# OSOceanAcoustics/echopype

Hardware: AMD Instinct MI355X
Metric: range-samples/sec through compute_Sv->compute_MVBS (higher is better)
Workload: dtype f64; 1 GPU; cfg5: EK60 CW 4x2000000x4096 in ping_time tiles, compute_Sv -> compute_MVBS(20s x 1m), Sv+MVBS out; tiles=8 x 250000 pings over 1 rank(s), route=compute_Sv -> compute_MVBS('1m','20s') per tile, collective=none at 1 rank, tile_streams=2

## Files before the change

### echopype_amd/csrc/epa_internal.h

```cpp
#pragma once
#include <cstdlib>
#include <hip/hip_runtime.h>

#include <atomic>

#include <cmath>
#include <cstdarg>
#include <cstdint>
#include <cstdio>

#include "echopype_amd.h"

namespace epa {

void set_error(const char* fmt, ...);

#define EPA_CHECK_ARG(cond, ...)       \
  do {                                 \
    if (!(cond)) {                     \
      ::epa::set_error(__VA_ARGS__);   \
      return EPA_EINVAL;               \
    }                                  \
  } while (0)

#define EPA_CHECK_HIP(expr)                                                              \
  do {                                                                                   \
    hipError_t _e = (expr);                                                              \
    if (_e != hipSuccess) {                                                              \
      ::epa::set_error("%s failed: %s (%s:%d)", #expr, hipGetErrorString(_e), __FILE__,  \
                       __LINE__);                                                        \
      return EPA_EHIP;                                                                   \
    }                                                                                    \
  } while (0)

template <typename T>
struct type_tag {
  using type = T;
};

template <typename T>
constexpr int dtype_of = sizeof(T) == 8 ? EPA_F64 : EPA_F32;

inline bool is_real(int dtype) { return dtype == EPA_F32 || dtype == EPA_F64; }

#define EPA_CHECK_REAL(who, dtype) EPA_CHECK_ARG(::epa::is_real(dtype), "%s: bad dtype %d", who, dtype)
#define EPA_CHECK_REAL_OUT(who, dtype) EPA_CHECK_ARG(::epa::is_real(dtype), "%s: bad output dtype %d", who, dtype)

template <typename F>
int dispatch_real(const char* who, int dtype, F&& f) {
  if (dtype == EPA_F64) return f(type_tag<double>{});
  if (dtype == EPA_F32) return f(type_tag<float>{});
  set_error("%s: bad dtype %d", who, dtype);
  return EPA_EINVAL;
}

extern std::atomic<bool> g_trace_on;
void note_launch(const char* what);
void note_range_stats_filled(int filled);

void note_seen(const char* what);

inline int check_launch(const char* what) {
  if (g_trace_on.load(std::memory_order_relaxed)) note_launch(what);
  note_seen(what);
  hipError_t e = hipGetLastError();
  if (e != hipSuccess) {
    set_error("launch of %s failed: %s", what, hipGetErrorString(e));
    return EPA_EHIP;
  }
  return EPA_OK;
}

constexpr int kBlock = 256;
constexpr int kMinmaxMaxGrid = 1024;

inline bool al16(const void* p) { return p == nullptr || (reinterpret_cast<uintptr_t>(p) & 15u) == 0; }

template <typename T>
struct M;
template <>
struct M<double> {
  static __device__ __forceinline__ double log10(double x) { return ::log10(x); }
  static __device__ __forceinline__ double exp10(double x) { return ::exp10(x); }
  static __device__ __forceinline__ double nan() { return __builtin_nan(""); }
};
template <>
struct M<float> {
  static __device__ __forceinline__ float log10(float x) { return ::log10f(x); }
  static __device__ __forceinline__ float exp10(float x) { return ::exp10f(x); }
  static __device__ __forceinline__ float nan() { return __builtin_nanf(""); }
};

struct CoefRow {
  double ra, rb, r0, shift, alpha2, A0, g, d;
};
static_assert(sizeof(CoefRow) == EPA_NCOEF * sizeof(double), "coef row layout");

__device__ __forceinline__ int xcd_contiguous(int x, int n) {
  const int per = n >> 3;
  return x < per * 8 ? (x & 7) * per + (x >> 3) : x;
}
inline bool xcd_map_enabled() {
  static const bool on = [] {
    const char* e = getenv("EPA_XCD_MAP");
    return !(e && e[0] == '0');
  }();
  return on;
}

__device__ __forceinline__ int range_bin_index(double x, double bin, double inv_bin, int nbins,
                                               bool closed_right) {
  if (!(x == x)) return -1;
  double t = x * inv_bin;
  if (!(t > -2.0)) return -1;
  if (t > (double)nbins + 2.0) return -1;
  int i;
  if (!closed_right) {
    i = (int)floor(t);
    if (x < (double)i * bin) --i;
    else if (x >= (double)(i + 1) * bin) ++i;
  } else {
    i = (int)ceil(t) - 1;
    if (x <= (double)i * bin) --i;
    else if (x > (double)(i + 1) * bin) ++i;
  }
  return (i >= 0 && i < nbins) ? i : -1;
}

__device__ __forceinline__ double row_range(const CoefRow& r, int s) {
  return ((double)s * r.ra) * r.rb + r.r0;
}

__device__ __forceinline__ double depth_of(double scale, double offset, double range) {
#pragma clang fp contract(off)
  const double prod = scale * range;
  return offset + prod;
}
__device__ __forceinline__ float depth_of(float scale, float offset, float range) {
#pragma clang fp contract(off)
  const float prod = scale * range;
  return offset + prod;
}

namespace scratch {
size_t sv_power_stats_workspace(long long S, long long, long long);
size_t depth_rows_workspace(long long, long long, long long);
size_t nanminmax_workspace(long long, long long, long long);
size_t range_step_mean_workspace(long long C, long long P, long long);
size_t sv_complex_cw_stats_workspace(long long, long long, long long);
size_t sv_complex_fft_workspace(long long W, long long P, long long S);
size_t splitbeam_complex_fft_workspace(long long n, long long, long long);
size_t sv_mvbs_fused_depth_stats(long long, long long, long long);
size_t apply_masks_workspace(long long, long long, long long);
size_t pool_sv_sum_ws(long long C, long long P, long long S);
size_t pool_sv_cnt_ws(long long C, long long P, long long S);
size_t pool_sv_value_ws_mean(long long C, long long P, long long S);
size_t pool_sv_value_ws_median(long long C, long long S, long long);
size_t nasc_workspace(long long C, long long n_dbins, long long n_rbins);
size_t seafloor_state(long long, long long, long long);
size_t seafloor_angle_mask_work(long long P, long long R, long long);
size_t seafloor_median_hist(long long, long long, long long);
size_t shoal_state(long long, long long, long long);
size_t shoal_echoview_link_queue(long long, long long, long long);
size_t transient_fielding_todo(long long C, long long P, long long);
size_t transient_fielding_count(long long, long long, long long);
size_t transient_matecho_s_hi(long long C, long long P, long long);
size_t transient_matecho_flag(long long C, long long P, long long);
size_t time_rebuild_tile_workspace(long long N, long long, long long);
size_t regrid_mask_out(long long G, long long n_tbins, long long n_rbins);
}

#define EPA_CHECK_SCRATCH(who, what, used, have)                                                              \
  EPA_CHECK_ARG((size_t)(used) <= (size_t)(have), "%s: internal error: the launch plan writes %zu bytes of %s, sized %zu", \
                who, (size_t)(used), what, (size_t)(have))

}

int epa_rows_piece_launch(const float* mask_raw, const void* x, const double* coef, const double* scale,
                          const double* offset, long long rows, int S, void* out, int dtype, double* workspace,
                          double* stats_out, hipStream_t st);
int epa_minmax_final(const double* part, int nparts, double* out, hipStream_t st);
int epa_minmax_keys_init(unsigned long long* keys, hipStream_t st);
int epa_minmax_keys_decode(double* keys, hipStream_t st);

int epa_fused_fast_path(const void* raw, int raw_is_i16, const int32_t* n_valid, const double* coef,
                        int C, int P, int S, double nspread,
                        unsigned cal_flags, const int32_t* bin_start, int n_tbins, double range_bin,
                        int n_rbins, unsigned bin_flags, double fill_value, void* sv_out,
                        void* mvbs_out, void* sum_out, uint32_t* cnt_out, int dtype,
                        size_t lds_bytes, unsigned cnt_off, unsigned long long* rmax_key,
                        unsigned long long* rstat, const double* dscale, const double* doffset, void* depth_out,
                        hipStream_t st);
int epa_mvbs_rows_fast_path(const void* sv, const double* coef, int C, int P, int S, const int32_t* bin_start,
                            int n_tbins, double range_bin, int n_rbins, int as_stored, double fill_value,
                            void* mvbs_out, void* sum_out, uint32_t* cnt_out, int dtype, size_t lds_bytes,
                            unsigned cnt_off, hipStream_t st);
int epa_chain_fast_pass1(const float* raw, const double* coef, const double* alpha2, int C, int P, int S,
                         double nspread, int ping_num, int rsn, int ping_phase, double noise_max, void* sv_out,
                         double* noise_out, double* edge_sum_out, uint32_t* edge_cnt_out,
                         unsigned long long* rmax_key, unsigned long long* rstat, int dtype, hipStream_t st);
int epa_chain_fast_pass2(const float* raw, const double* coef, const double* alpha2, const double* noise, int C,
                         int P, int S, double nspread, int ping_num, int ping_phase, double snr,
                         const int32_t* bin_start, int n_tbins, double range_bin, int n_rbins, double fill_value,
                         void* noise_out, void* corr_out, void* mvbs_out, void* sum_out, uint32_t* cnt_out, int dtype,
                         size_t lds_acc_bytes, unsigned cnt_off, unsigned long long* mm_keys, hipStream_t st);
```

### echopype_amd/csrc/fused_sv_mvbs.hip

```cpp
#include <hip/amd_detail/amd_hip_unsafe_atomics.h>

#include <cstdlib>
#include <type_traits>

#include "fast_math.h"
#include "ordered_key.h"
#include "sample_math.h"

namespace epa_fused {

constexpr int VEC = 4;
constexpr int kChunk = epa::kBlock * VEC;

struct Args {
  int P, S, n_tbins, n_rbins;
  double range_bin, inv_range_bin;
  double nspread, fill_value;
  unsigned guard, mask_range, skipna, closed_right;
  unsigned cnt_off, tab_off;
  unsigned long long* rmax_key;
  unsigned long long* rstat;
  int xcd_map;
  int flagged_only;
  const double* dscale;
  const double* doffset;
  void* depth_out;
};

using epa::kKeyNoMax;
using epa::kKeyNoMin;
using epa::key_value;
using epa::lds_add;
using epa::ordered_key;
using epa::vmax_num;
using epa::vmin_num;

template <typename T>
__device__ __noinline__ T log10_slow(T x) {
  return epa::M<T>::log10(x);
}

template <typename T>
struct Column {
  double sra;
  double blo, bhi;
  T nL;
  T acc_sum;
  int acc_rb;
  uint32_t acc_cnt;
  __device__ __forceinline__ void init() {
    sra = 0.0; blo = 1.0; bhi = 0.0; nL = epa::M<T>::nan(); acc_sum = (T)0; acc_rb = -1; acc_cnt = 0u;
  }
  __device__ __forceinline__ void flush(T* lsum, uint32_t* lcnt, uint32_t n_clean) {
    const uint32_t n = acc_cnt + n_clean;
    if (acc_rb >= 0 && n > 0u) {
      lds_add(lsum + acc_rb, acc_sum);
      atomicAdd(lcnt + acc_rb, n);
    }
  }
  __device__ __forceinline__ void rebin(double x, bool valid, double bin, double inv_bin, int n_rbins, T* lsum,
                                        uint32_t* lcnt, uint32_t n_clean) {
    const int rb = valid ? epa::range_bin_index(x, bin, inv_bin, n_rbins, false) : -1;
    if (rb != acc_rb) {
      flush(lsum, lcnt, n_clean);
      acc_rb = rb;
      acc_sum = (T)0;
      acc_cnt = 0u - n_clean;
    }
    blo = rb >= 0 ? (double)rb * bin : 1.0;
    bhi = rb >= 0 ? (double)(rb + 1) * bin : 0.0;
  }
};

__device__ __forceinline__ double lin_bins(double u, const double* __restrict__ tab) {
  constexpr double K256 = 85.04135922911648, Z = 0.0027076061740622863;
  constexpr double C1 = Z, C2 = Z * Z / 2.0, C3 = Z * Z * Z / 6.0;
  const double t = u * K256;
  const double m = __builtin_rint(t);
  const double r = fma(u, K256, -m);
  double p = fma(r, C3, C2);
  p = fma(p, r, C1);
  p = fma(p, r, 1.0);
  const int mi = __double2int_rz(m);
  return ldexp(p * tab[mi & 255], mi >> 8);
}
__device__ __forceinline__ float lin_bins(float u, const double*) { return ::exp10f(u * 0.1f); }

template <typename T, bool STATS>
__device__ __forceinline__ T process_sample(Column<T>& c, float raw, const epa::CoefRow& r, double r0v, T g, T a2,
                                            T A0v, T nL, T nspread, double bin, double inv_bin, int n_rbins,
                                            const double* tab, T* lsum, uint32_t* lcnt, double& xmax, double& xmin,
                                            unsigned& nnan, uint32_t n_clean) {
  const T NaN = epa::M<T>::nan();
  const double x = fma(c.sra, r.rb, r0v);
  if (STATS) {
    if (raw == raw) {
      xmax = vmax_num(xmax, x);
      xmin = vmin_num(xmin, x);
    }
    nnan += (unsigned)__builtin_popcountll(__ballot(raw != raw));
  }
  const double rtd = x - r.shift;
  const T rt = (T)rtd;
  const bool pos = rtd > 0.0;
  T s1 = fma(g, (T)raw, nL);
  if (pos & !(nL > -(T)__builtin_inf()))
    s1 = fma(g, (T)raw, nspread * (log10_slow<T>(rt) - log10_slow<T>((T)(r.ra * r.rb))));
  s1 = pos ? s1 : NaN;
  const T sv = s1 + fma(a2, rt, A0v);
  const T v = epa::lin_from_db_lean(sv, tab);
  const bool same = (x >= c.blo) & (x < c.bhi);
  if (!same) c.rebin(x, raw == raw, bin, inv_bin, n_rbins, lsum, lcnt, n_clean);
  c.acc_sum += vmax_num(v, (T)0);
  c.acc_cnt += v == v ? 1u : 0u;
  return sv;
}

template <typename T, bool STATS, bool WRITE_SV, int DEPTH>
__device__ __forceinline__ void process_pair(Column<T>& c0, Column<T>& c1, float2 in, bool clean, const epa::CoefRow& r,
                                             double r0v, T g, T a2, T A0v, T nL0, T nL1, T nspread, double bin,
                                             double inv_bin, int n_rbins, const double* tab, T* lsum, uint32_t* lcnt,
                                             T* __restrict__ sv_dst, double& xmax, double& xmin, unsigned& nnan,
                                             uint32_t n_clean, double& xfirst, double& xlast, T dsc, T dof,
                                             T* __restrict__ depth_dst, double sra0, double sra1) {
  const double e0 = fma(sra0, r.rb, r0v), e1 = fma(sra1, r.rb, r0v);
  const double rtd0 = e0 - r.shift, rtd1 = e1 - r.shift;
  T d0 = (T)0, d1 = (T)0;
  if (DEPTH) {
    d0 = epa::depth_of(dsc, dof, (T)e0);
    d1 = epa::depth_of(dsc, dof, (T)e1);
  }
  const double x0 = DEPTH ? (double)d0 : e0, x1 = DEPTH ? (double)d1 : e1;
  const T rt0 = (T)rtd0, rt1 = (T)rtd1;
  T s10 = fma(g, (T)in.x, nL0), s11 = fma(g, (T)in.y, nL1);
  if (!clean) {
    const T NaN = epa::M<T>::nan();
    const bool pos0 = rtd0 > 0.0, pos1 = rtd1 > 0.0;
    if (pos0 & !(nL0 > -(T)__builtin_inf()))
      s10 = fma(g, (T)in.x, nspread * (log10_slow<T>(rt0) - log10_slow<T>((T)(r.ra * r.rb))));
    if (pos1 & !(nL1 > -(T)__builtin_inf()))
      s11 = fma(g, (T)in.y, nspread * (log10_slow<T>(rt1) - log10_slow<T>((T)(r.ra * r.rb))));
    s10 = pos0 ? s10 : NaN;
    s11 = pos1 ? s11 : NaN;
    if (STATS) {
      if (in.x == in.x) {
        xmax = vmax_num(xmax, x0);
        xmin = vmin_num(xmin, x0);
      }
      if (in.y == in.y) {
        xmax = vmax_num(xmax, x1);
        xmin = vmin_num(xmin, x1);
      }
      nnan += (unsigned)__builtin_popcountll(__ballot((in.x != in.x) | (x0 != x0))) +
              (unsigned)__builtin_popcountll(__ballot((in.y != in.y) | (x1 != x1)));
    }
    if (DEPTH == 2) {
      d0 = epa::nan_where_nan(d0, in.x);
      d1 = epa::nan_where_nan(d1, in.y);
    }
  }
  if (DEPTH == 2) epa::store_nt2(depth_dst, d0, d1);
  const T sv0 = s10 + fma(a2, rt0, A0v), sv1 = s11 + fma(a2, rt1, A0v);
  if (WRITE_SV) {
#ifndef EPA_PLAIN_STORES
    epa::store_nt2(sv_dst, sv0, sv1);
#else
    const T o[2] = {sv0, sv1};
    epa::store_vec<T, 2>(sv_dst, o);
#endif
  }
  T v0 = lin_bins(sv0, tab), v1 = lin_bins(sv1, tab);
  if (!clean) {
    if (__builtin_expect(__builtin_isinf(sv0), 0)) v0 = sv0 < (T)0 ? (T)0 : sv0;
    if (__builtin_expect(__builtin_isinf(sv1), 0)) v1 = sv1 < (T)0 ? (T)0 : sv1;
  }
  if (!((x0 >= c0.blo) & (x0 < c0.bhi))) c0.rebin(x0, in.x == in.x, bin, inv_bin, n_rbins, lsum, lcnt, n_clean);
  if (!((x1 >= c1.blo) & (x1 < c1.bhi))) c1.rebin(x1, in.y == in.y, bin, inv_bin, n_rbins, lsum, lcnt, n_clean);
  if (clean) {
    c0.acc_sum += v0;
    c1.acc_sum += v1;
  } else {
    c0.acc_sum += vmax_num(v0, (T)0);
    c1.acc_sum += vmax_num(v1, (T)0);
    c0.acc_cnt += v0 == v0 ? 1u : 0u;
    c1.acc_cnt += v1 == v1 ? 1u : 0u;
  }
  xfirst = x0;
  xlast = x1;
}

__device__ __forceinline__ bool not_finite(float x) { return __builtin_amdgcn_classf(x, 0x207); }

template <typename RawT>
struct PingLoad;
template <>
struct PingLoad<float> {
  float2 a, b;
  __device__ __forceinline__ PingLoad() : a(make_float2(0.f, 0.f)), b(make_float2(0.f, 0.f)) {}
  __device__ __forceinline__ void issue(const float* __restrict__ row, int sA, int sB, bool hasB, int, int) {
    a = *reinterpret_cast<const float2*>(row + sA);
    if (hasB) b = *reinterpret_cast<const float2*>(row + sB);
  }
  __device__ __forceinline__ void resolve(float2& A, float2& B, int, int, int, bool) const {
    A = a;
    B = b;
  }
};
template <>
struct PingLoad<int16_t> {
  unsigned a, b;
  __device__ __forceinline__ PingLoad() : a(0u), b(0u) {}
  __device__ __forceinline__ void issue(const int16_t* __restrict__ row, int sA, int sB, bool hasB, int, int) {
    a = *reinterpret_cast<const unsigned*>(row + sA);
    if (hasB) b = *reinterpret_cast<const unsigned*>(row + sB);
  }
  static __device__ __forceinline__ float2 unpack(unsigned w, int s, int n_valid) {
    constexpr float kIndex2Power = 0.011758984205624266f;
    const float nanv = __builtin_nanf("");
    const float x = (float)(short)(w & 0xffffu), y = (float)(short)(w >> 16);
    return make_float2(s < n_valid ? x * kIndex2Power : nanv, s + 1 < n_valid ? y * kIndex2Power : nanv);
  }
  static __device__ __forceinline__ float2 unpack_all(unsigned w) {
    constexpr float kIndex2Power = 0.011758984205624266f;
    return make_float2((float)(short)(w & 0xffffu) * kIndex2Power, (float)(short)(w >> 16) * kIndex2Power);
  }
  __device__ __forceinline__ void resolve(float2& A, float2& B, int sA, int sB, int nv, bool full) const {
    if (full) {
      A = unpack_all(a);
      B = unpack_all(b);
    } else {
      A = unpack(a, sA, nv);
      B = unpack(b, sB, nv);
    }
  }
};

#ifndef EPA_FUSED_MIN_WAVES
#define EPA_FUSED_MIN_WAVES 1
#endif
#ifndef EPA_FUSED_LEAN
#define EPA_FUSED_LEAN 1
#endif
__device__ __forceinline__ double uniform(double v) {
  return __hiloint2double(__builtin_amdgcn_readfirstlane(__double2hiint(v)), __builtin_amdgcn_readfirstlane(__double2loint(v)));
}

__device__ __forceinline__ bool finite_bits(double v) { return (__double2hiint(v) & 0x7ff00000) != 0x7ff00000; }

template <typename T, typename RawT, bool WRITE_SV, bool RMAX, int DEPTH>
__global__ __launch_bounds__(epa::kBlock, EPA_FUSED_MIN_WAVES > 4 ? EPA_FUSED_MIN_WAVES : 4) void fused_sv_mvbs_kernel(
    const RawT* __restrict__ raw, const int32_t* __restrict__ n_valid,
    const epa::CoefRow* __restrict__ coef,
    const int32_t* __restrict__ bin_start, T* __restrict__ sv_out, T* __restrict__ mvbs_out,
    T* __restrict__ sum_out, uint32_t* __restrict__ cnt_out, const double* __restrict__ dscale,
    const double* __restrict__ doffset, Args a) {
  extern __shared__ __attribute__((aligned(16))) unsigned char smem[];
  T* lsum = reinterpret_cast<T*>(smem);
  uint32_t* lcnt = reinterpret_cast<uint32_t*>(smem + a.cnt_off);
  const epa::MathTabs mt = epa::build_math_tabs(smem + a.tab_off);
  const double* tab = mt.exp2_tab;
  constexpr bool NL_LDS = RMAX || sizeof(T) == 8;
  __shared__ T col_nL[NL_LDS ? kChunk : 1];
  constexpr bool SRA_LDS = (RMAX || std::is_same<RawT, int16_t>::value) && sizeof(T) == 8;
  __shared__ double col_sra[SRA_LDS ? kChunk : 1];
  __shared__ unsigned long long wg_keys[2];
  __shared__ unsigned wg_nnan;
  if (RMAX && threadIdx.x == 0) {
    wg_keys[0] = kKeyNoMax;
    wg_keys[1] = kKeyNoMin;
    wg_nnan = 0u;
  }

  const int c = blockIdx.y, tb = a.xcd_map ? epa::xcd_contiguous(blockIdx.x, a.n_tbins) : (int)blockIdx.x;
  const int S = a.S, n_rbins = a.n_rbins;
  const bool extra = tb == a.n_tbins;
  if (extra && !WRITE_SV) return;
  const int nseg = extra ? 2 : 1;
  for (int i = threadIdx.x; i < n_rbins; i += epa::kBlock) {
    lsum[i] = (T)0;
    lcnt[i] = 0u;
  }
  __syncthreads();

  const T nspread = (T)a.nspread;
  const double bin = a.range_bin, inv_bin = a.inv_range_bin;
  const epa::CoefRow* __restrict__ rowp0 = coef + (size_t)c * a.P;
  const RawT* __restrict__ raw_c = raw + (size_t)c * a.P * S;
  const int32_t* __restrict__ nv_c = n_valid ? n_valid + (size_t)c * a.P : nullptr;
  T* __restrict__ sv_c = WRITE_SV ? sv_out + (size_t)c * a.P * S : nullptr;
  T* __restrict__ dp_c = DEPTH == 2 ? reinterpret_cast<T*>(a.depth_out) + (size_t)c * a.P * S : nullptr;
  const double* __restrict__ dsc_c = DEPTH ? dscale + (size_t)c * a.P : nullptr;
  const double* __restrict__ dof_c = DEPTH ? doffset + (size_t)c * a.P : nullptr;
  const int wave = __builtin_amdgcn_readfirstlane((int)(threadIdx.x >> 6)), lane = threadIdx.x & 63;
  double xmax = -__builtin_inf(), xmin = __builtin_inf();
  unsigned nnan = 0u;

  for (int seg = 0; seg < nseg; ++seg) {
  const int pb = extra ? (seg == 0 ? 0 : bin_start[a.n_tbins]) : bin_start[tb];
  const int pe = extra ? (seg == 0 ? bin_start[0] : a.P) : bin_start[tb + 1];
  for (int chunk0 = 0; chunk0 < S; chunk0 += kChunk) {
    const int sA = chunk0 + wave * 256 + 2 * lane;
    const int sB = sA + 128;
    if (sA >= S) continue;
    const bool hasB = sB < S;
    Column<T> col[VEC];
#pragma unroll
    for (int j = 0; j < VEC; ++j) col[j].init();
    const int eA = wave * 256 + 2 * lane;
    if (NL_LDS) {
      col_nL[eA] = col_nL[eA + 1] = col_nL[eA + 128] = col_nL[eA + 129] = epa::M<T>::nan();
    }
    long long dcur = 0x7ff8dead00000001ll, racur = 0x7ff8dead00000002ll;
    uint32_t n_clean = 0u;
    bool plain = false;
    const int s4 = chunk0 + wave * 256 + 4 * lane;
    PingLoad<RawT> nxt;
    epa::CoefRow nxtR = rowp0[pb < pe ? pb : 0];
    double nxtDs = 1.0, nxtDo = 0.0;
    if (DEPTH) {
      nxtDs = uniform(dsc_c[pb < pe ? pb : 0]);
      nxtDo = uniform(dof_c[pb < pe ? pb : 0]);
    }
    int nxtNv = nv_c && pb < pe ? nv_c[pb] : S;
    if (pb < pe) nxt.issue(raw_c + (size_t)pb * S, sA, sB, hasB, s4, S);
    for (int p = pb; p < pe; ++p) {
      const epa::CoefRow r = nxtR;
      const double curDs = nxtDs, curDo = nxtDo;
      const size_t row_off = (size_t)p * S;
      const int nv = nxtNv;
      float2 inA, inB;
      const bool full = nv_c != nullptr && nv >= chunk0 + wave * 256 + 256;
      nxt.resolve(inA, inB, sA, sB, nv, full);
      if (p + 1 < pe) {
        nxtR = rowp0[p + 1];
        if (nv_c) nxtNv = nv_c[p + 1];
        if (DEPTH) {
          nxtDs = uniform(dsc_c[p + 1]);
          nxtDo = uniform(dof_c[p + 1]);
        }
        nxt.issue(raw_c + row_off + S, sA, sB, hasB, s4, S);
      }
      if (!((__double_as_longlong(r.d) == dcur) & (__double_as_longlong(r.ra) == racur))) {
        dcur = __double_as_longlong(r.d);
        racur = __double_as_longlong(r.ra);
        bool fin = true;
        for (int j = 0; j < VEC; ++j) {
          const double sj = (double)((j < 2 ? sA : sB) + (j & 1));
          const T nl = nspread * log10_slow<T>((T)(sj - r.d));
          if (NL_LDS) col_nL[eA + (j < 2 ? 0 : 128) + (j & 1)] = nl;
          else col[j].nL = nl;
          if (SRA_LDS) col_sra[eA + (j < 2 ? 0 : 128) + (j & 1)] = sj * r.ra;
          else col[j].sra = sj * r.ra;
          fin = fin & ((j >= 2 && !hasB) | (fabs(nl) < (T)__builtin_inf()));
        }
        plain = __ballot(!fin) == 0ull;
      }
      const T g = (T)r.g, a2 = (T)r.alpha2;
      T A0 = (T)r.A0;
      double r0v = r.r0;
      asm volatile("" : "+v"(A0), "+v"(r0v));
      bool clean = false;
#if EPA_FUSED_LEAN
      {
        const double xa = fma(SRA_LDS ? col_sra[eA] : col[0].sra, r.rb, r0v);
        bool bad = !(xa - r.shift > 0.0);
        if (!full) bad = bad | not_finite(inA.x) | not_finite(inA.y) | not_finite(inB.x) | not_finite(inB.y);
        bool kpos = (__double2hiint(r.ra) > 0) & (__double2hiint(r.rb) > 0) & finite_bits(r.g) & finite_bits(r.A0) &
                    finite_bits(r.alpha2);
        if (DEPTH) kpos = kpos & finite_bits(curDs) & finite_bits(curDo);
        clean = plain & kpos & (__ballot(bad) == 0ull);
      }
#endif
      const T dsc = (T)curDs, dof = (T)curDo;
      double xf, xl, xdummy;
      process_pair<T, RMAX, WRITE_SV, DEPTH>(col[0], col[1], inA, clean, r, r0v, g, a2, A0, NL_LDS ? col_nL[eA] : col[0].nL,
                                             NL_LDS ? col_nL[eA + 1] : col[1].nL, nspread, bin, inv_bin, n_rbins, tab, lsum,
                                             lcnt, WRITE_SV ? sv_c + row_off + sA : nullptr, xmax, xmin, nnan, n_clean, xf,
                                             xl, dsc, dof, DEPTH == 2 ? dp_c + row_off + sA : nullptr,
                                             SRA_LDS ? col_sra[eA] : col[0].sra, SRA_LDS ? col_sra[eA + 1] : col[1].sra);
      if (hasB)
        process_pair<T, RMAX, WRITE_SV, DEPTH>(col[2], col[3], inB, clean, r, r0v, g, a2, A0,
                                               NL_LDS ? col_nL[eA + 128] : col[2].nL, NL_LDS ? col_nL[eA + 129] : col[3].nL,
                                               nspread, bin, inv_bin, n_rbins, tab, lsum, lcnt,
                                               WRITE_SV ? sv_c + row_off + sB : nullptr, xmax, xmin, nnan, n_clean, xdummy,
                                               xl, dsc, dof, DEPTH == 2 ? dp_c + row_off + sB : nullptr,
                                               SRA_LDS ? col_sra[eA + 128] : col[2].sra,
                                               SRA_LDS ? col_sra[eA + 129] : col[3].sra);
      if (clean) {
        if (RMAX) {
          if (DEPTH) {
            xmin = vmin_num(vmin_num(xmin, xf), xl);
            xmax = vmax_num(vmax_num(xmax, xf), xl);
          } else {
            xmin = vmin_num(xmin, xf);
            xmax = vmax_num(xmax, xl);
          }
        }
        ++n_clean;
      }
    }
#pragma unroll
    for (int j = 0; j < VEC; ++j) col[j].flush(lsum, lcnt, n_clean);
  }
  }
  if (RMAX) {
#pragma unroll
    for (int o = 32; o > 0; o >>= 1) xmax = fmax(xmax, __shfl_down(xmax, o, 64));
#pragma unroll
    for (int o = 32; o > 0; o >>= 1) xmin = fmin(xmin, __shfl_down(xmin, o, 64));
    if (lane == 0) {
      if (xmax > -__builtin_inf()) atomicMax(&wg_keys[0], ordered_key(xmax));
      if (xmin < __builtin_inf()) atomicMin(&wg_keys[1], ordered_key(xmin));
      if (nnan > 0u) atomicAdd(&wg_nnan, nnan);
    }
    __syncthreads();
    if (threadIdx.x == 0) {
      const unsigned long long kmax = wg_keys[0], kmin = wg_keys[1];
      if (kmax != kKeyNoMax) atomicMax(a.rmax_key, kmax);
      if (a.rstat) {
        if (kmin != kKeyNoMin) atomicMin(a.rstat, kmin);
        if (wg_nnan > 0u) atomicAdd(a.rstat + 1, (unsigned long long)wg_nnan);
      }
    }
  }
  if (extra) return;
  __syncthreads();
  const size_t cell0 = ((size_t)c * a.n_tbins + tb) * n_rbins;
  T* out = mvbs_out + cell0;
  T* gsum = sum_out ? sum_out + cell0 : nullptr;
  uint32_t* gcnt = cnt_out ? cnt_out + cell0 : nullptr;
  for (int i = threadIdx.x; i < n_rbins; i += epa::kBlock) {
    const uint32_t n = lcnt[i];
    const T s = lsum[i];
    out[i] = n > 0u ? (T)10 * epa::M<T>::log10(s / (T)n) : (T)a.fill_value;
    if (gsum) gsum[i] = s;
    if (gcnt) gcnt[i] = n;
  }
}

template <typename T, typename RawT>
int launch(Args& a, const RawT* raw, const int32_t* n_valid, const double* coef, const int32_t* bin_start,
           void* sv_out, void* mvbs_out, void* sum_out, uint32_t* cnt_out, int C, size_t lds_bytes,
           hipStream_t st) {
  const dim3 grid((unsigned)a.n_tbins + 1u, (unsigned)C);
  a.tab_off = (unsigned)((lds_bytes + 15) & ~(size_t)15);
  lds_bytes = a.tab_off + epa::kMathTabBytes;
  a.xcd_map = epa::xcd_map_enabled() ? 1 : 0;
#define EPA_FL(W, R) EPA_FLD(W, R, 0)
#define EPA_FLD(W, R, D)                                                                       \
  do {                                                                                         \
    auto kern = fused_sv_mvbs_kernel<T, RawT, W, R, D>;                                        \
    if (lds_bytes > 64 * 1024)                                                                 \
      EPA_CHECK_HIP(hipFuncSetAttribute(reinterpret_cast<const void*>(kern),                   \
                                        hipFuncAttributeMaxDynamicSharedMemorySize,            \
                                        (int)lds_bytes));                                      \
    hipLaunchKernelGGL(kern, grid, dim3(epa::kBlock), lds_bytes, st, raw, n_valid,             \
                       reinterpret_cast<const epa::CoefRow*>(coef), bin_start, (T*)sv_out,     \
                       (T*)mvbs_out, (T*)sum_out, cnt_out, a.dscale, a.doffset, a);            \
  } while (0)
  if (a.dscale) {
    if constexpr (std::is_same<RawT, float>::value) {
      if (a.depth_out) EPA_FLD(true, true, 2);
      else if (sv_out) EPA_FLD(true, true, 1);
      else EPA_FLD(false, true, 1);
    } else {
      epa::set_error("epa_sv_mvbs_fused_depth: float power samples only");
      return EPA_EUNSUPPORTED;
    }
  } else if (a.rmax_key) {
    if (sv_out) EPA_FL(true, true); else EPA_FL(false, true);
  } else {
    if (sv_out) EPA_FL(true, false); else EPA_FL(false, false);
  }
#undef EPA_FLD
#undef EPA_FL
  return epa::check_launch("fused_sv_mvbs_kernel");
}

__global__ __launch_bounds__(epa::kBlock) void selftest_lin_kernel(const double* __restrict__ u,
                                                                   double* __restrict__ out,
                                                                   size_t n) {
  __shared__ __attribute__((aligned(16))) unsigned char tabs[epa::kMathTabBytes];
  const epa::MathTabs mt = epa::build_math_tabs(tabs);
  __syncthreads();
  for (size_t i = (size_t)blockIdx.x * blockDim.x + threadIdx.x; i < n;
       i += (size_t)gridDim.x * blockDim.x)
    out[i] = epa::lin_from_db(u[i], mt.exp2_tab);
}

__global__ __launch_bounds__(epa::kBlock) void selftest_log_kernel(const double* __restrict__ x,
                                                                   double* __restrict__ out,
                                                                   size_t n) {
  __shared__ __attribute__((aligned(16))) unsigned char tabs[epa::kMathTabBytes];
  const epa::MathTabs mt = epa::build_math_tabs(tabs);
  __syncthreads();
  for (size_t i = (size_t)blockIdx.x * blockDim.x + threadIdx.x; i < n;
       i += (size_t)gridDim.x * blockDim.x)
    out[i] = epa::fast_log10(x[i], mt.log_tab);
}

__global__ __launch_bounds__(epa::kBlock) void selftest_log_inl_kernel(const double* __restrict__ x,
                                                                       double* __restrict__ out, size_t n) {
  __shared__ __attribute__((aligned(16))) unsigned char tabs[epa::kMathTabBytes];
  const epa::MathTabs mt = epa::build_math_tabs(tabs);
  __syncthreads();
  for (size_t i = (size_t)blockIdx.x * blockDim.x + threadIdx.x; i < n;
       i += (size_t)gridDim.x * blockDim.x)
    out[i] = epa::fast_log10_inl<false>(x[i], mt.log_tab);
}

template <typename T>
struct SvColumn {
  double sra, blo, bhi;
  T acc_sum;
  int acc_rb;
  uint32_t acc_cnt;
  __device__ __forceinline__ void init() { sra = 0.0; blo = 1.0; bhi = 0.0; acc_sum = (T)0; acc_rb = -1; acc_cnt = 0u; }
  __device__ __forceinline__ void flush(T* lsum, uint32_t* lcnt) {
    if (acc_rb >= 0 && acc_cnt > 0u) {
      lds_add(lsum + acc_rb, acc_sum);
      atomicAdd(lcnt + acc_rb, acc_cnt);
    }
  }
};

template <typename T, bool AS_STORED>
__device__ __forceinline__ void bin_sv_sample(SvColumn<T>& c, T sv, const epa::CoefRow& r, double bin, double inv_bin,
                                              int n_rbins, const double* tab, T* lsum, uint32_t* lcnt) {
  const double x0 = c.sra * r.rb + r.r0;
  const double x = AS_STORED ? (double)(T)x0 : x0;
  const T v = epa::lin_from_db(sv, tab);
  const bool same = (x >= c.blo) & (x < c.bhi);
  if (!same) {
    const int rb = (x == x) ? epa::range_bin_index(x, bin, inv_bin, n_rbins, false) : -1;
    if (rb != c.acc_rb) {
      c.flush(lsum, lcnt);
      c.acc_rb = rb;
      c.acc_sum = (T)0;
      c.acc_cnt = 0u;
    }
    c.blo = rb >= 0 ? (double)rb * bin : 1.0;
    c.bhi = rb >= 0 ? (double)(rb + 1) * bin : 0.0;
  }
  const bool take = (c.acc_rb >= 0) & (v == v);
  c.acc_sum += take ? v : (T)0;
  c.acc_cnt += take ? 1u : 0u;
}

constexpr int kFixedPings = 512;
using LeftToRows = epa::LeftMark<0x7ff8dead0c0ffee2ull, 0x7fcdead2u>;

template <typename T, bool AS_STORED>
__global__ __launch_bounds__(epa::kBlock, sizeof(T) == 8 ? 6 : 8) void mvbs_of_sv_fixed_kernel(
    const T* __restrict__ sv, const epa::CoefRow* __restrict__ coef, const int32_t* __restrict__ bin_start,
    T* __restrict__ mvbs_out, T* __restrict__ sum_out, uint32_t* __restrict__ cnt_out, Args a) {
  typedef T T2 __attribute__((ext_vector_type(2)));
  extern __shared__ __attribute__((aligned(16))) unsigned char smem[];
  T* lsum = reinterpret_cast<T*>(smem);
  uint32_t* lcnt = reinterpret_cast<uint32_t*>(smem + a.cnt_off);
  const epa::MathTabs mt = epa::build_math_tabs(smem + a.tab_off);
  const double* tab = mt.exp2_tab;
  __shared__ int differs;
  __shared__ unsigned long long rb_lo_key, rb_hi_key;
  const int c = blockIdx.y, tb = a.xcd_map ? epa::xcd_contiguous(blockIdx.x, a.n_tbins) : (int)blockIdx.x;
  const int S = a.S, n_rbins = a.n_rbins;
  const int pb = bin_start[tb], pe = bin_start[tb + 1], np = pe - pb;
  const size_t cell0 = ((size_t)c * a.n_tbins + tb) * n_rbins;
  for (int i = threadIdx.x; i < n_rbins; i += epa::kBlock) {
    lsum[i] = (T)0;
    lcnt[i] = 0u;
  }
  if (threadIdx.x == 0) {
    differs = np > kFixedPings ? 1 : 0;
    rb_lo_key = kKeyNoMin;
    rb_hi_key = kKeyNoMax;
  }
  __syncthreads();
  const epa::CoefRow* __restrict__ rowp0 = coef + (size_t)c * a.P;
  const epa::CoefRow r = rowp0[np > 0 ? pb : 0];
  for (int i = threadIdx.x; i < min(np, kFixedPings); i += epa::kBlock) {
    const epa::CoefRow ri = rowp0[pb + i];
    if (!((ri.ra == r.ra) & (ri.r0 == r.r0) & (ri.rb == ri.rb) & (ri.ra > 0.0))) differs = 1;
    atomicMin(&rb_lo_key, ordered_key(ri.rb));
    atomicMax(&rb_hi_key, ordered_key(ri.rb));
  }
  __syncthreads();
  if (differs) {
    if (threadIdx.x == 0) LeftToRows::mark(mvbs_out + cell0);
    return;
  }
  const double rb_lo = key_value(rb_lo_key), rb_hi = key_value(rb_hi_key);
  const double bin = a.range_bin, inv_bin = a.inv_range_bin;
  const T* __restrict__ sv_c = sv + (size_t)c * a.P * S;
  const int wave = threadIdx.x >> 6, lane = threadIdx.x & 63;
  auto range_of = [&](int sx, double rb) {
    const double x0 = ((double)sx * r.ra) * rb + r.r0;
    return AS_STORED ? (double)(T)x0 : x0;
  };
  for (int chunk0 = 0; chunk0 < S; chunk0 += kChunk) {
    const int sA = chunk0 + wave * 256 + 2 * lane;
    const int sB = sA + 128;
    if (sA >= S) continue;
    const bool hasB = sB < S;
    int rbin[VEC];
    T acc_sum[VEC];
    uint32_t acc_cnt[VEC];
    unsigned fixed = 0;
#pragma unroll
    for (int j = 0; j < VEC; ++j) {
      const int sx = (j < 2 ? sA : sB) + (j & 1);
      const int b_lo = epa::range_bin_index(range_of(sx, rb_lo), bin, inv_bin, n_rbins, false);
      const int b_hi = epa::range_bin_index(range_of(sx, rb_hi), bin, inv_bin, n_rbins, false);
      rbin[j] = b_lo;
      if (b_lo == b_hi) fixed |= 1u << j;
      acc_sum[j] = (T)0;
      acc_cnt[j] = 0u;
    }
    T2 nA0 = {(T)0, (T)0}, nB0 = nA0, nA1 = nA0, nB1 = nA0;
    if (np > 0) {
      nA0 = *reinterpret_cast<const T2*>(sv_c + (size_t)pb * S + sA);
      if (hasB) nB0 = *reinterpret_cast<const T2*>(sv_c + (size_t)pb * S + sB);
    }
    if (np > 1) {
      nA1 = *reinterpret_cast<const T2*>(sv_c + (size_t)(pb + 1) * S + sA);
      if (hasB) nB1 = *reinterpret_cast<const T2*>(sv_c + (size_t)(pb + 1) * S + sB);
    }
    for (int p = pb; p < pe; ++p) {
      const T2 inA = nA0, inB = nB0;
      nA0 = nA1;
      nB0 = nB1;
      if (p + 2 < pe) {
        const T* nx = sv_c + (size_t)(p + 2) * S;
        nA1 = *reinterpret_cast<const T2*>(nx + sA);
        if (hasB) nB1 = *reinterpret_cast<const T2*>(nx + sB);
      }
      const T in[VEC] = {inA.x, inA.y, inB.x, inB.y};
#pragma unroll
      for (int j = 0; j < VEC; ++j) {
        if (j >= 2 && !hasB) break;
        const T v = epa::lin_from_db_lean(in[j], tab);
        acc_sum[j] += vmax_num(v, (T)0);
        acc_cnt[j] += v == v ? 1u : 0u;
      }
    }
#pragma unroll
    for (int j = 0; j < VEC; ++j) {
      if (((fixed >> j) & 1u) != 0u && rbin[j] >= 0 && acc_cnt[j] > 0u) {
        lds_add(lsum + rbin[j], acc_sum[j]);
        atomicAdd(lcnt + rbin[j], acc_cnt[j]);
      }
    }
    const unsigned loose = (~fixed) & (hasB ? 0xfu : 0x3u);
    if (__ballot(loose != 0u) != 0ull) {
      const int nact = (int)__popcll(__ballot(true));
#pragma unroll 1
      for (int j = 0; j < VEC; ++j) {
        unsigned long long todo = __ballot(((loose >> j) & 1u) != 0u);
        while (todo != 0ull) {
          const int src = __ffsll((long long)todo) - 1;
          todo &= todo - 1ull;
          const int sx = chunk0 + wave * 256 + 2 * src + (j < 2 ? 0 : 128) + (j & 1);
          for (int p = pb + lane; p < pe; p += nact) {
            const T v = epa::lin_from_db_lean(sv_c[(size_t)p * S + sx], tab);
            const double x = range_of(sx, rowp0[p].rb);
            const int rb = epa::range_bin_index(x, bin, inv_bin, n_rbins, false);
            if ((rb >= 0) & (v == v)) {
              lds_add(lsum + rb, v);
              atomicAdd(lcnt + rb, 1u);
            }
          }
        }
      }
    }
  }
  __syncthreads();
  T* out = mvbs_out + cell0;
  T* gsum = sum_out ? sum_out + cell0 : nullptr;
  uint32_t* gcnt = cnt_out ? cnt_out + cell0 : nullptr;
  for (int i = threadIdx.x; i < n_rbins; i += epa::kBlock) {
    const uint32_t n = lcnt[i];
    const T s = lsum[i];
    out[i] = n > 0u ? (T)10 * epa::M<T>::log10(s / (T)n) : (T)a.fill_value;
    if (gsum) gsum[i] = s;
    if (gcnt) gcnt[i] = n;
  }
}

template <typename T, bool AS_STORED>
__global__ __launch_bounds__(epa::kBlock, EPA_FUSED_MIN_WAVES) void mvbs_of_sv_rows_kernel(
    const T* __restrict__ sv, const epa::CoefRow* __restrict__ coef, const int32_t* __restrict__ bin_start,
    T* __restrict__ mvbs_out, T* __restrict__ sum_out, uint32_t* __restrict__ cnt_out, Args a) {
  typedef T T2 __attribute__((ext_vector_type(2)));
  extern __shared__ __attribute__((aligned(16))) unsigned char smem[];
  T* lsum = reinterpret_cast<T*>(smem);
  uint32_t* lcnt = reinterpret_cast<uint32_t*>(smem + a.cnt_off);
  const epa::MathTabs mt = epa::build_math_tabs(smem + a.tab_off);
  const double* tab = mt.exp2_tab;
  const int c = blockIdx.y, tb = a.xcd_map ? epa::xcd_contiguous(blockIdx.x, a.n_tbins) : (int)blockIdx.x;
  const int S = a.S, n_rbins = a.n_rbins;
  if (a.flagged_only && !LeftToRows::is_marked(mvbs_out + ((size_t)c * a.n_tbins + tb) * n_rbins)) return;
  for (int i = threadIdx.x; i < n_rbins; i += epa::kBlock) {
    lsum[i] = (T)0;
    lcnt[i] = 0u;
  }
  __syncthreads();
  const double bin = a.range_bin, inv_bin = a.inv_range_bin;
  const epa::CoefRow* __restrict__ rowp0 = coef + (size_t)c * a.P;
  const T* __restrict__ sv_c = sv + (size_t)c * a.P * S;
  const int wave = threadIdx.x >> 6, lane = threadIdx.x & 63;
  const int pb = bin_start[tb], pe = bin_start[tb + 1];
  for (int chunk0 = 0; chunk0 < S; chunk0 += kChunk) {
    const int sA = chunk0 + wave * 256 + 2 * lane;
    const int sB = sA + 128;
    if (sA >= S) continue;
    const bool hasB = sB < S;
    SvColumn<T> col[VEC];
#pragma unroll
    for (int j = 0; j < VEC; ++j) col[j].init();
    double racur = __builtin_nan("");
    T2 nA = {(T)0, (T)0}, nB = {(T)0, (T)0};
    epa::CoefRow nxtR = rowp0[pb < pe ? pb : 0];
    if (pb < pe) {
      nA = *reinterpret_cast<const T2*>(sv_c + (size_t)pb * S + sA);
      if (hasB) nB = *reinterpret_cast<const T2*>(sv_c + (size_t)pb * S + sB);
    }
    for (int p = pb; p < pe; ++p) {
      const epa::CoefRow r = nxtR;
      const T2 inA = nA, inB = nB;
      if (p + 1 < pe) {
        nxtR = rowp0[p + 1];
        const T* nx = sv_c + (size_t)(p + 1) * S;
        nA = *reinterpret_cast<const T2*>(nx + sA);
        if (hasB) nB = *reinterpret_cast<const T2*>(nx + sB);
      }
      if (!(r.ra == racur)) {
        racur = r.ra;
        for (int j = 0; j < VEC; ++j) col[j].sra = (double)((j < 2 ? sA : sB) + (j & 1)) * r.ra;
      }
      bin_sv_sample<T, AS_STORED>(col[0], inA.x, r, bin, inv_bin, n_rbins, tab, lsum, lcnt);
      bin_sv_sample<T, AS_STORED>(col[1], inA.y, r, bin, inv_bin, n_rbins, tab, lsum, lcnt);
      if (hasB) {
        bin_sv_sample<T, AS_STORED>(col[2], inB.x, r, bin, inv_bin, n_rbins, tab, lsum, lcnt);
        bin_sv_sample<T, AS_STORED>(col[3], inB.y, r, bin, inv_bin, n_rbins, tab, lsum, lcnt);
      }
    }
#pragma unroll
    for (int j = 0; j < VEC; ++j) col[j].flush(lsum, lcnt);
  }
  __syncthreads();
  const size_t cell0 = ((size_t)c * a.n_tbins + tb) * n_rbins;
  T* out = mvbs_out + cell0;
  T* gsum = sum_out ? sum_out + cell0 : nullptr;
  uint32_t* gcnt = cnt_out ? cnt_out + cell0 : nullptr;
  for (int i = threadIdx.x; i < n_rbins; i += epa::kBlock) {
    const uint32_t n = lcnt[i];
    const T s = lsum[i];
    out[i] = n > 0u ? (T)10 * epa::M<T>::log10(s / (T)n) : (T)a.fill_value;
    if (gsum) gsum[i] = s;
    if (gcnt) gcnt[i] = n;
  }
}

template <typename T>
int launch_sv_rows(Args& a, const void* sv, const double* coef, const int32_t* bin_start, void* mvbs_out, void* sum_out,
                   uint32_t* cnt_out, int C, size_t lds_bytes, bool as_stored, hipStream_t st) {
  const dim3 grid((unsigned)a.n_tbins, (unsigned)C);
  a.tab_off = (unsigned)((lds_bytes + 15) & ~(size_t)15);
  lds_bytes = a.tab_off + epa::kMathTabBytes;
  a.xcd_map = epa::xcd_map_enabled() ? 1 : 0;
  static const bool fixed_off = [] {
    const char* e = getenv("EPA_MVBS_FIXED");
    return e && e[0] == '0';
  }();
#define EPA_SR(KERN, AS)                                                                                 \
  do {                                                                                                   \
    auto kern = KERN<T, AS>;                                                                             \
    if (lds_bytes > 64 * 1024)                                                                           \
      EPA_CHECK_HIP(hipFuncSetAttribute(reinterpret_cast<const void*>(kern),                             \
                                        hipFuncAttributeMaxDynamicSharedMemorySize, (int)lds_bytes));    \
    hipLaunchKernelGGL(kern, grid, dim3(epa::kBlock), lds_bytes, st, (const T*)sv,                       \
                       reinterpret_cast<const epa::CoefRow*>(coef), bin_start, (T*)mvbs_out, (T*)sum_out, \
                       cnt_out, a);                                                                      \
  } while (0)
  a.flagged_only = 0;
  if (!fixed_off) {
    if (as_stored) EPA_SR(mvbs_of_sv_fixed_kernel, true); else EPA_SR(mvbs_of_sv_fixed_kernel, false);
    if (int rc = epa::check_launch("mvbs_of_sv_fixed_kernel")) return rc;
    a.flagged_only = 1;
  }
  if (as_stored) EPA_SR(mvbs_of_sv_rows_kernel, true); else EPA_SR(mvbs_of_sv_rows_kernel, false);
#undef EPA_SR
  return epa::check_launch("mvbs_of_sv_rows_kernel");
}

}

int epa_mvbs_rows_fast_path(const void* sv, const double* coef, int C, int P, int S, const int32_t* bin_start,
                            int n_tbins, double range_bin, int n_rbins, int as_stored, double fill_value,
                            void* mvbs_out, void* sum_out, uint32_t* cnt_out, int dtype, size_t lds_bytes,
                            unsigned cnt_off, hipStream_t st) {
  epa_fused::Args a{};
  a.P = P; a.S = S; a.n_tbins = n_tbins; a.n_rbins = n_rbins;
  a.range_bin = range_bin; a.inv_range_bin = 1.0 / range_bin;
  a.fill_value = fill_value;
  a.skipna = 1;
  a.cnt_off = cnt_off;
  return epa::dispatch_real("epa_mvbs_rows_fast_path", dtype, [&](auto tag) {
    return epa_fused::launch_sv_rows<typename decltype(tag)::type>(a, sv, coef, bin_start, mvbs_out, sum_out, cnt_out, C,
                                                                   lds_bytes, as_stored != 0, st);
  });
}

extern "C" int epa_selftest_lin_from_db(const double* u, double* out, size_t n, epa_stream_t stream) {
  EPA_CHECK_ARG(u && out, "epa_selftest_lin_from_db: NULL array argument");
  if (n == 0) return EPA_OK;
  const size_t blocks = (n + epa::kBlock - 1) / epa::kBlock;
  hipLaunchKernelGGL(epa_fused::selftest_lin_kernel, dim3((unsigned)(blocks < 1024 ? blocks : 1024)),
                     dim3(epa::kBlock), 0, (hipStream_t)stream, u, out, n);
  return epa::check_launch("selftest_lin_kernel");
}

extern "C" int epa_selftest_log10(const double* x, double* out, size_t n, epa_stream_t stream) {
  EPA_CHECK_ARG(x && out, "epa_selftest_log10: NULL array argument");
  if (n == 0) return EPA_OK;
  const size_t blocks = (n + epa::kBlock - 1) / epa::kBlock;
  hipLaunchKernelGGL(epa_fused::selftest_log_kernel, dim3((unsigned)(blocks < 1024 ? blocks : 1024)),
                     dim3(epa::kBlock), 0, (hipStream_t)stream, x, out, n);
  return epa::check_launch("selftest_log_kernel");
}

extern "C" int epa_selftest_log10_inline(const double* x, double* out, size_t n, epa_stream_t stream) {
  EPA_CHECK_ARG(x && out, "epa_selftest_log10_inline: NULL array argument");
  if (n == 0) return EPA_OK;
  const size_t blocks = (n + epa::kBlock - 1) / epa::kBlock;
  hipLaunchKernelGGL(epa_fused::selftest_log_inl_kernel, dim3((unsigned)(blocks < 1024 ? blocks : 1024)),
                     dim3(epa::kBlock), 0, (hipStream_t)stream, x, out, n);
  return epa::check_launch("selftest_log_inl_kernel");
}

int epa_fused_fast_path(const void* raw, int raw_is_i16, const int32_t* n_valid, const double* coef,
                        int C, int P, int S, double nspread,
                        unsigned cal_flags, const int32_t* bin_start, int n_tbins, double range_bin,
                        int n_rbins, unsigned bin_flags, double fill_value, void* sv_out,
                        void* mvbs_out, void* sum_out, uint32_t* cnt_out, int dtype,
                        size_t lds_bytes, unsigned cnt_off, unsigned long long* rmax_key,
                        unsigned long long* rstat, const double* dscale, const double* doffset, void* depth_out,
                        hipStream_t st) {
  epa_fused::Args a{};
  a.dscale = dscale; a.doffset = doffset; a.depth_out = dscale ? depth_out : nullptr;
  a.rmax_key = rmax_key;
  a.rstat = rmax_key ? rstat : nullptr;
  a.P = P; a.S = S; a.n_tbins = n_tbins; a.n_rbins = n_rbins;
  a.range_bin = range_bin; a.inv_range_bin = 1.0 / range_bin;
  a.nspread = nspread; a.fill_value = fill_value;
  a.guard = (cal_flags & EPA_FLAG_GUARD_POS) != 0;
  a.mask_range = (cal_flags & EPA_FLAG_MASK_RANGE) != 0;
  a.skipna = (bin_flags & EPA_BIN_SKIPNA) != 0;
  a.closed_right = (bin_flags & EPA_BIN_CLOSED_RIGHT) != 0;
  a.cnt_off = cnt_off;
  return epa::dispatch_real("epa_fused_fast_path", dtype, [&](auto tag) {
    using T = typename decltype(tag)::type;
    if (raw_is_i16)
      return epa_fused::launch<T, int16_t>(a, reinterpret_cast<const int16_t*>(raw), n_valid, coef, bin_start, sv_out,
                                           mvbs_out, sum_out, cnt_out, C, lds_bytes, st);
    return epa_fused::launch<T, float>(a, reinterpret_cast<const float*>(raw), n_valid, coef, bin_start, sv_out, mvbs_out,
                                       sum_out, cnt_out, C, lds_bytes, st);
  });
}
```

Before: 483.9 billion range-samples/s.

## Flatten channel into grid x and add staggered chunk/ping walk start options

Collapses the 2D (time-bin, channel) grid into a 1D grid in which consecutive workgroups on each XCD cycle through channels before moving to the next time bin. This is meant to spread the channels of one time bin across compute units and keep XCD-local L2 traffic contiguous. It also adds optional, environment-selected rotation of the starting range chunk and ping per workgroup to de-correlate memory access; by default only the channel interleave is on. The cost is extra index arithmetic and a rotated ping order, which changes the floating-point accumulation order in the MVBS sums.

```diff
diff --git a/echopype_amd/csrc/epa_internal.h b/echopype_amd/csrc/epa_internal.h
--- a/echopype_amd/csrc/epa_internal.h
+++ b/echopype_amd/csrc/epa_internal.h
@@ -106,6 +106,25 @@
     return !(e && e[0] == '0');
   }();
   return on;
+}
+
+struct WalkStart {
+  int chunk, ping;
+};
+__device__ __forceinline__ WalkStart walk_start(int i, int n_chunks, int n_pings) {
+  WalkStart w{0, 0};
+  if (n_chunks > 1) {
+    w.chunk = i % n_chunks;
+    i /= n_chunks;
+  }
+  if (n_pings > 1) w.ping = i % n_pings;
+  return w;
+}
+constexpr int kWalkChunk = 1, kWalkPing = 2, kWalkChannels = 4;
+constexpr int kWalkDefault = kWalkChannels;
+inline int walk_start_mode() {
+  const char* e = getenv("EPA_WALK_START");
+  return e && e[0] ? atoi(e) & 7 : kWalkDefault;
 }
 
 __device__ __forceinline__ int range_bin_index(double x, double bin, double inv_bin, int nbins,
diff --git a/echopype_amd/csrc/fused_sv_mvbs.hip b/echopype_amd/csrc/fused_sv_mvbs.hip
--- a/echopype_amd/csrc/fused_sv_mvbs.hip
+++ b/echopype_amd/csrc/fused_sv_mvbs.hip
@@ -25,6 +25,7 @@
   const double* dscale;
   const double* doffset;
   void* depth_out;
+  int walk, C;
 };
 
 using epa::kKeyNoMax;
@@ -271,7 +272,14 @@
     wg_nnan = 0u;
   }
 
-  const int c = blockIdx.y, tb = a.xcd_map ? epa::xcd_contiguous(blockIdx.x, a.n_tbins) : (int)blockIdx.x;
+  int c = blockIdx.y, tb = a.xcd_map ? epa::xcd_contiguous(blockIdx.x, a.n_tbins) : (int)blockIdx.x;
+  const int wg_i = (int)(blockIdx.x >> 3);
+  if (a.walk & epa::kWalkChannels) {
+    const int id = (int)blockIdx.x, per = a.xcd_map ? a.n_tbins >> 3 : 0, full = per * 8 * a.C;
+    const int k = id < full ? id >> 3 : id - full;
+    c = k % a.C;
+    tb = (id < full ? (id & 7) * per : per * 8) + k / a.C;
+  }
   const int S = a.S, n_rbins = a.n_rbins;
   const bool extra = tb == a.n_tbins;
   if (extra && !WRITE_SV) return;
@@ -298,7 +306,13 @@
   for (int seg = 0; seg < nseg; ++seg) {
   const int pb = extra ? (seg == 0 ? 0 : bin_start[a.n_tbins]) : bin_start[tb];
   const int pe = extra ? (seg == 0 ? bin_start[0] : a.P) : bin_start[tb + 1];
-  for (int chunk0 = 0; chunk0 < S; chunk0 += kChunk) {
+  const int n_chunks = (S + kChunk - 1) / kChunk;
+  epa::WalkStart ws = extra ? epa::WalkStart{0, 0} : epa::walk_start(wg_i, n_chunks, pe - pb);
+  if (!(a.walk & epa::kWalkChunk)) ws.chunk = 0;
+  if (!(a.walk & epa::kWalkPing)) ws.ping = 0;
+  const int p0 = pb + ws.ping;
+  for (int ck = 0; ck < n_chunks; ++ck) {
+    const int chunk0 = (ck + ws.chunk - (ck + ws.chunk >= n_chunks ? n_chunks : 0)) * kChunk;
     const int sA = chunk0 + wave * 256 + 2 * lane;
     const int sB = sA + 128;
     if (sA >= S) continue;
@@ -315,15 +329,16 @@
     bool plain = false;
     const int s4 = chunk0 + wave * 256 + 4 * lane;
     PingLoad<RawT> nxt;
-    epa::CoefRow nxtR = rowp0[pb < pe ? pb : 0];
+    epa::CoefRow nxtR = rowp0[pb < pe ? p0 : 0];
     double nxtDs = 1.0, nxtDo = 0.0;
     if (DEPTH) {
-      nxtDs = uniform(dsc_c[pb < pe ? pb : 0]);
-      nxtDo = uniform(dof_c[pb < pe ? pb : 0]);
-    }
-    int nxtNv = nv_c && pb < pe ? nv_c[pb] : S;
-    if (pb < pe) nxt.issue(raw_c + (size_t)pb * S, sA, sB, hasB, s4, S);
-    for (int p = pb; p < pe; ++p) {
+      nxtDs = uniform(dsc_c[pb < pe ? p0 : 0]);
+      nxtDo = uniform(dof_c[pb < pe ? p0 : 0]);
+    }
+    int nxtNv = nv_c && pb < pe ? nv_c[p0] : S;
+    if (pb < pe) nxt.issue(raw_c + (size_t)p0 * S, sA, sB, hasB, s4, S);
+    int p = p0;
+    for (int left = pe - pb; left > 0; --left) {
       const epa::CoefRow r = nxtR;
       const double curDs = nxtDs, curDo = nxtDo;
       const size_t row_off = (size_t)p * S;
@@ -331,14 +346,15 @@
       float2 inA, inB;
       const bool full = nv_c != nullptr && nv >= chunk0 + wave * 256 + 256;
       nxt.resolve(inA, inB, sA, sB, nv, full);
-      if (p + 1 < pe) {
-        nxtR = rowp0[p + 1];
-        if (nv_c) nxtNv = nv_c[p + 1];
+      const int pn = p + 1 < pe ? p + 1 : pb;
+      if (left > 1) {
+        nxtR = rowp0[pn];
+        if (nv_c) nxtNv = nv_c[pn];
         if (DEPTH) {
-          nxtDs = uniform(dsc_c[p + 1]);
-          nxtDo = uniform(dof_c[p + 1]);
+          nxtDs = uniform(dsc_c[pn]);
+          nxtDo = uniform(dof_c[pn]);
         }
-        nxt.issue(raw_c + row_off + S, sA, sB, hasB, s4, S);
+        nxt.issue(raw_c + (size_t)pn * S, sA, sB, hasB, s4, S);
       }
       if (!((__double_as_longlong(r.d) == dcur) & (__double_as_longlong(r.ra) == racur))) {
         dcur = __double_as_longlong(r.d);
@@ -398,6 +414,7 @@
         }
         ++n_clean;
       }
+      p = pn;
     }
 #pragma unroll
     for (int j = 0; j < VEC; ++j) col[j].flush(lsum, lcnt, n_clean);
@@ -442,7 +459,11 @@
 int launch(Args& a, const RawT* raw, const int32_t* n_valid, const double* coef, const int32_t* bin_start,
            void* sv_out, void* mvbs_out, void* sum_out, uint32_t* cnt_out, int C, size_t lds_bytes,
            hipStream_t st) {
-  const dim3 grid((unsigned)a.n_tbins + 1u, (unsigned)C);
+  a.walk = epa::walk_start_mode();
+  a.C = C;
+  if (((long long)a.n_tbins + 1) * C > 0x7fffffffll) a.walk &= ~epa::kWalkChannels;
+  const dim3 grid = (a.walk & epa::kWalkChannels) ? dim3(((unsigned)a.n_tbins + 1u) * (unsigned)C)
+                                                  : dim3((unsigned)a.n_tbins + 1u, (unsigned)C);
   a.tab_off = (unsigned)((lds_bytes + 15) & ~(size_t)15);
   lds_bytes = a.tab_off + epa::kMathTabBytes;
   a.xcd_map = epa::xcd_map_enabled() ? 1 : 0;
```

Result: slower. 431.5 billion range-samples/s (-10.8%).
